# althonos/pyhmmer

Hardware: AMD Instinct MI355X
Metric: GCUPS (DP cells/s) + seqs/s for hmmsearch, Pfam-A vs proteome, 1/2/4/8 GPUs (higher is better)
Workload: dtype u8/i16 filters (MSV, Viterbi), f32 Forward/Backward

## Files before the change

### include/p7x.h

```cpp
#ifndef P7X_H
#define P7X_H

#include <stddef.h>
#include <stdint.h>

#ifdef __cplusplus
extern "C" {
#endif

#define P7X_ABI_VERSION 8

enum {
  P7X_OK = 0, P7X_EMEM = 5, P7X_EFORMAT = 7, P7X_EINVAL = 11, P7X_ERANGE = 16, P7X_ENORESULT = 19,
  P7X_ENODEVICE = 100, P7X_EDEVICE = 101
};

enum { P7X_RNA = 1, P7X_DNA = 2, P7X_AMINO = 3 };
enum { P7X_SEARCH_SEQS = 0, P7X_SCAN_MODELS = 1 };
enum { P7X_ZSETBY_NTARGETS = 0, P7X_ZSETBY_OPTION = 1, P7X_ZSETBY_FILEINFO = 2 };
enum { P7X_MMU = 0, P7X_MLAMBDA, P7X_VMU, P7X_VLAMBDA, P7X_FTAU, P7X_FLAMBDA };
enum { P7X_GA1 = 0, P7X_GA2, P7X_TC1, P7X_TC2, P7X_NC1, P7X_NC2 };
#define P7X_CUTOFF_UNSET (-99999.0f)
#define P7X_EVPARAM_UNSET (-99999.0f)
enum { P7X_IS_INCLUDED = 1, P7X_IS_REPORTED = 2, P7X_IS_NEW = 4, P7X_IS_DROPPED = 8, P7X_IS_DUPLICATE = 16 };
// ... 119 lines not shown
  int64_t seqidx;
  int32_t window_length;
  double sortkey;
  float score, pre_score, sum_score;
  double lnP, pre_lnP, sum_lnP;
  float nexpected;
  int32_t nregions, nclustered, noverlaps, nenvelopes, ndom;
  uint32_t flags;
  int32_t nreported, nincluded, best_domain;
} p7x_hit;

typedef struct p7x_tophits p7x_tophits;

int p7x_search_block(const p7x_pipeline_cfg *cfg, const p7x_oprofile *om, const float *bg_f,
                     const p7x_seqdb *db, const char *const *names, const char *const *accs,
                     const char *const *descs, p7x_tophits **out);

typedef struct p7x_pending p7x_pending;
int  p7x_search_block_begin(const p7x_pipeline_cfg *cfg, const p7x_oprofile *om, const float *bg_f,
                            const p7x_seqdb *db, p7x_pending **out);
int  p7x_search_block_finish(p7x_pending *pending, const char *const *names, const char *const *accs,
                             const char *const *descs, p7x_tophits **out);
void p7x_pending_destroy(p7x_pending *pending);
int  p7x_search_block_enqueue(const p7x_pipeline_cfg *cfg, const p7x_oprofile *om, const float *bg_f,
                              const p7x_seqdb *db, p7x_pending **out);
int  p7x_search_block_wait(p7x_pending *pending);
int  p7x_search_batch_enqueue(const p7x_pipeline_cfg *cfg, const p7x_oprofile *const *oms, size_t nq, const float *bg_f,
                              const p7x_seqdb *db, p7x_pending **out);
int  p7x_search_batch_finish(p7x_pending *pending, const char *const *names, const char *const *accs,
                             const char *const *descs, p7x_tophits **outs);
size_t p7x_pending_nqueries(const p7x_pending *pending);
int  p7x_debug_log_of_float(int device, const float *in, float *out, size_t n);
int  p7x_debug_memory_stats(int device, int64_t out[4]);
int  p7x_debug_choice(const float *p, int n, uint32_t x, int *via_thresholds, int *via_fchoose);
int  p7x_debug_order_spread(const p7x_oprofile *om, const uint8_t *dsq1, int32_t L, int32_t i, int32_t j, int multihit, double *out12);
int  p7x_debug_parser_rows(const p7x_oprofile *om, const uint8_t *dsq1, int32_t L, float *fx, float *bx);
int64_t p7x_debug_ssv_tables(const p7x_oprofile *om, int pair, int32_t *R, int32_t *pair_slack, uint32_t *tab4q, size_t cap_words);
int  p7x_debug_set_option(const char *name, int value);
int  p7x_debug_ensemble(const p7x_oprofile *om, const p7x_seqdb *db, int64_t target, int32_t i, int32_t j, uint32_t seed,
                        int use_device, int32_t *ndom, int32_t *dom, int32_t dom_cap, float *n2, int32_t *status);
int  p7x_search_batch_raw(const p7x_pipeline_cfg *cfg, const p7x_oprofile *const *oms, size_t nq, const float *bg_f,
                          const p7x_seqdb *db, int32_t *xJ, int32_t *xC, uint8_t *stage);

int p7x_search_longtargets(const p7x_pipeline_cfg *cfg, const p7x_oprofile *om, int device,
                           const uint8_t *dsq, const int64_t *offsets, const int64_t *lengths, size_t n,
                           const char *const *names, const char *const *accs, const char *const *descs, p7x_tophits **out);
int p7x_longtargets_release_resident(int device, uint64_t key);
int64_t p7x_ssv_longtarget_seeds(const p7x_pipeline_cfg *cfg, const p7x_oprofile *om, int device, const uint8_t *dsq, int64_t L,
                                 int complement, int64_t *seeds, size_t cap);
int p7x_longtarget_from_seeds(const p7x_pipeline_cfg *cfg, const p7x_oprofile *om,
                              const uint8_t *dsq, const int64_t *offsets, const int64_t *lengths, size_t n,
                              const char *const *names, const char *const *accs, const char *const *descs,
                              const int64_t *seed_target, const int64_t *seed_block, const int32_t *seed_strand,
                              const int64_t *seeds, size_t nseeds, p7x_tophits **out);

int p7x_forward_parser_exact(const p7x_oprofile *om, const uint8_t *dsq, int32_t L, float *sc);

int p7x_scan_collect(p7x_tophits *const *per_model, size_t nmodels, const p7x_pipeline_cfg *cfg, size_t nseqs,
                     const char *const *seq_names, const char *const *seq_accs, const char *const *seq_descs,
                     const int32_t *seq_lengths, p7x_tophits **out);
typedef struct p7x_scan_accum p7x_scan_accum;
int  p7x_scan_accum_create(const p7x_pipeline_cfg *cfg, size_t nseqs, const char *const *seq_names, const char *const *seq_accs,
                           const char *const *seq_descs, const int32_t *seq_lengths, p7x_scan_accum **out);
int  p7x_scan_accum_add(p7x_scan_accum *acc, p7x_tophits *const *per_model, size_t nmodels);
int  p7x_scan_accum_add_indexed(p7x_scan_accum *acc, p7x_tophits *const *per_model, const int64_t *model_index, size_t nmodels);
int  p7x_debug_tophits_set_stages(p7x_tophits *th, const uint8_t *stage, size_t n);
// ... 92 lines not shown
```

### pyhmmer_amd/_lib.py

```python
from __future__ import annotations

import ctypes as C
import os
import shutil
import subprocess
from pathlib import Path

_PKG = Path(__file__).resolve().parent
_ROOT = _PKG.parent
CSRC = _PKG / "csrc"
LIB_PATH = _PKG / "libp7x.so"

SOURCES = ["p7x_profile.cpp", "p7x_device.hip", "p7x_devmem.hip", "p7x_devimage.hip", "p7x_msv.hip", "p7x_vitfwd.hip", "p7x_vitpk.hip", "p7x_fwdpk.hip", "p7x_envelope.hip", "p7x_ensemble.hip", "p7x_ssvlong.hip", "p7x_longtarget.hip",
           "p7x_envscore.hip", "p7x_pipeline.hip", "p7x_domaindef.cpp", "p7x_longtarget_host.cpp", "p7x_tophits.cpp", "p7x_align.hip", "p7x_tracealign.cpp", "p7x_builder.cpp", "p7x_calibrate.hip"]


def _hipcc() -> str:
    for cand in (os.environ.get("HIPCC"), shutil.which("hipcc"), "/opt/rocm/bin/hipcc"):
        if cand and os.path.exists(cand):
            return cand
    raise RuntimeError("hipcc not found (need ROCm; set HIPCC=/path/to/hipcc)")


ISA_CHECKED = ("p7x_msv.hip", "p7x_envelope.hip")
# ... 163 lines not shown
    "p7x_pipeline_cfg_default": (None, [C.POINTER(PipelineCfg)]),
    "p7x_search_block": (C.c_int, [C.POINTER(PipelineCfg), _VP, _VP, _VP, _VP, _VP, _VP, C.POINTER(_VP)]),
    "p7x_postprocess_targets": (C.c_int, [C.POINTER(PipelineCfg), _VP, _VP, _VP, _VP, C.c_size_t, _VP, C.c_size_t, _VP, _VP, _VP,
                                          _VP, _VP, _VP, _VP, _VP, C.POINTER(_VP)]),
    "p7x_tophits_destroy": (None, [_VP]),
    "p7x_tophits_destroy_many": (None, [_VP, C.c_size_t]),
    "p7x_tophits_clone": (_VP, [_VP]),
    "p7x_tophits_nhits": (C.c_int64, [_VP]),
    "p7x_tophits_abc_type": (C.c_int, [_VP]),
    "p7x_tophits_get_counters": (C.c_int, [_VP, C.POINTER(Counters)]),
    "p7x_tophits_get_cfg": (C.c_int, [_VP, C.POINTER(PipelineCfg)]),
    "p7x_tophits_get_hit": (C.c_int, [_VP, C.c_int64, C.POINTER(HitRec)]),
    "p7x_tophits_get_domain": (C.c_int, [_VP, C.c_int64, C.c_int32, C.POINTER(DomainRec)]),
    "p7x_tophits_merge": (C.c_int, [_VP, _VP]),
    "p7x_tophits_serialize": (C.c_int64, [_VP, _VP, C.c_size_t]),
    "p7x_tophits_deserialize": (_VP, [_VP, C.c_size_t]),
    "p7x_tophits_sort_by_key": (C.c_int, [_VP]),
    "p7x_tophits_threshold": (C.c_int, [_VP]),
    "p7x_tophits_sort_by_seqidx": (C.c_int, [_VP]),
    "p7x_tophits_is_sorted": (C.c_int, [_VP, C.c_int]),
    "p7x_tophits_set_hit_flags": (C.c_int, [_VP, C.c_int64, C.c_uint32]),
    "p7x_tophits_set_hit_text": (C.c_int, [_VP, C.c_int64, C.c_int, C.c_char_p]),
    "p7x_tophits_get_timings": (C.c_int, [_VP, C.POINTER(C.c_double), C.c_int]),
    "p7x_search_block_begin": (C.c_int, [C.POINTER(PipelineCfg), _VP, _VP, _VP, C.POINTER(_VP)]),
    "p7x_search_block_enqueue": (C.c_int, [C.POINTER(PipelineCfg), _VP, _VP, _VP, C.POINTER(_VP)]),
    "p7x_search_block_wait": (C.c_int, [_VP]),
    "p7x_search_block_finish": (C.c_int, [_VP, _VP, _VP, _VP, C.POINTER(_VP)]),
    "p7x_pending_destroy": (None, [_VP]),
    "p7x_search_batch_enqueue": (C.c_int, [C.POINTER(PipelineCfg), C.POINTER(_VP), C.c_size_t, _VP, _VP, C.POINTER(_VP)]),
    "p7x_search_batch_finish": (C.c_int, [_VP, _VP, _VP, _VP, C.POINTER(_VP)]),
    "p7x_pending_nqueries": (C.c_size_t, [_VP]),
    "p7x_debug_log_of_float": (C.c_int, [C.c_int, _VP, _VP, C.c_size_t]),
    "p7x_debug_memory_stats": (C.c_int, [C.c_int, C.POINTER(C.c_int64)]),
    "p7x_debug_choice": (C.c_int, [_VP, C.c_int, C.c_uint32, _VP, _VP]),
    "p7x_debug_order_spread": (C.c_int, [_VP, _VP, C.c_int32, C.c_int32, C.c_int32, C.c_int, _VP]),
    "p7x_debug_parser_rows": (C.c_int, [_VP, _VP, C.c_int32, _VP, _VP]),
    "p7x_debug_ssv_tables": (C.c_int64, [_VP, C.c_int, _VP, _VP, _VP, C.c_size_t]),
    "p7x_debug_set_option": (C.c_int, [C.c_char_p, C.c_int]),
    "p7x_longtargets_release_resident": (C.c_int, [C.c_int, C.c_uint64]),
    "p7x_debug_ensemble": (C.c_int, [_VP, _VP, C.c_int64, C.c_int32, C.c_int32, C.c_uint32, C.c_int, _VP, _VP, C.c_int32, _VP, _VP]),
    "p7x_search_batch_raw": (C.c_int, [C.POINTER(PipelineCfg), C.POINTER(_VP), C.c_size_t, _VP, _VP, _VP, _VP, _VP]),
    "p7x_search_longtargets": (C.c_int, [C.POINTER(PipelineCfg), _VP, C.c_int, _VP, _VP, _VP, C.c_size_t, _VP, _VP, _VP, C.POINTER(_VP)]),
    "p7x_ssv_longtarget_seeds": (C.c_int64, [C.POINTER(PipelineCfg), _VP, C.c_int, _VP, C.c_int64, C.c_int, _VP, C.c_size_t]),
    "p7x_forward_parser_exact": (C.c_int, [_VP, _VP, C.c_int32, C.POINTER(C.c_float)]),
    "p7x_longtarget_from_seeds": (C.c_int, [C.POINTER(PipelineCfg), _VP, _VP, _VP, _VP, C.c_size_t, _VP, _VP, _VP, _VP, _VP, _VP, _VP,
                                            C.c_size_t, C.POINTER(_VP)]),
    "p7x_oprofile_write_pressed": (C.c_int, [_VP, C.POINTER(C.c_int64), _VP, C.c_size_t, C.POINTER(C.c_size_t), _VP, C.c_size_t,
                                             C.POINTER(C.c_size_t)]),
    "p7x_oprofile_read_pressed": (C.c_int, [_VP, C.c_size_t, _VP, C.c_size_t, _VP, C.POINTER(_VP), C.POINTER(C.c_size_t),
                                            C.POINTER(C.c_size_t), C.POINTER(C.c_int64)]),
    "p7x_oprofile_get_string": (C.c_int, [_VP, C.c_int, C.c_char_p, C.c_size_t]),
    "p7x_scan_collect": (C.c_int, [C.POINTER(_VP), C.c_size_t, C.POINTER(PipelineCfg), C.c_size_t, _VP, _VP, _VP, _VP, C.POINTER(_VP)]),
    "p7x_scan_accum_create": (C.c_int, [C.POINTER(PipelineCfg), C.c_size_t, _VP, _VP, _VP, _VP, C.POINTER(_VP)]),
    "p7x_scan_accum_add": (C.c_int, [_VP, C.POINTER(_VP), C.c_size_t]),
    "p7x_scan_accum_add_indexed": (C.c_int, [_VP, C.POINTER(_VP), C.POINTER(C.c_int64), C.c_size_t]),
    "p7x_debug_tophits_set_stages": (C.c_int, [_VP, _VP, C.c_size_t]),
    "p7x_scan_accum_finish": (C.c_int, [_VP, C.POINTER(_VP)]),
    "p7x_scan_accum_destroy": (None, [_VP]),
    "p7x_fasta_parse": (C.c_int, [_VP, C.c_size_t, _VP, C.POINTER(C.c_size_t), C.POINTER(C.c_size_t), C.POINTER(C.c_size_t),
                                  _VP, _VP, _VP, _VP, _VP, _VP, C.POINTER(C.c_size_t)]),
    "p7x_tracealign_compute": (C.c_int, [_VP, C.c_int, _VP, _VP, _VP, C.c_size_t, C.c_int, C.POINTER(_VP)]),
    "p7x_traces_count": (C.c_int64, [_VP]),
    "p7x_traces_nflagged": (C.c_int64, [_VP]),
    "p7x_traces_stats": (C.c_int, [_VP, _VP]),
    "p7x_traces_get": (C.c_int, [_VP, C.c_int64, C.POINTER(C.c_int32), C.POINTER(C.c_int32), C.POINTER(C.c_int32), _VP,
                                 C.POINTER(C.c_int32), C.POINTER(C.c_uint8)]),
# ... 64 lines not shown
```

### pyhmmer_amd/csrc/p7x_device.hip

```cpp
#include "p7x_device.hpp"
#include <cstdlib>
#include "p7x_kernels.hpp"
#include <algorithm>
#include <cmath>
#include <cstring>
#include <map>
#include <memory>

namespace p7x {

static std::mutex g_ctx_mu;
static std::map<int, std::unique_ptr<DeviceCtx>> g_ctx;

static int device_count_checked()
{
  int n = 0;
  if (hipGetDeviceCount(&n) != hipSuccess) { (void) hipGetLastError(); return 0; }
  return n;
}

static const int g_hw_queues_set = setenv("GPU_MAX_HW_QUEUES", "8", 0);

int create_tail_stream(DeviceCtx *ctx, bool high_priority, hipStream_t *out)
{
  (void) ctx;
  int least = 0, greatest = 0;
  P7X_HIP(hipDeviceGetStreamPriorityRange(&least, &greatest));
  P7X_HIP(hipStreamCreateWithPriority(out, hipStreamNonBlocking, high_priority ? greatest : least));
  return P7X_OK;
}

int get_ctx(int device, DeviceCtx **out)
{
  std::lock_guard<std::mutex> lk(g_ctx_mu);
  auto it = g_ctx.find(device);
  if (it != g_ctx.end()) { *out = it->second.get(); P7X_HIP(hipSetDevice(device)); return P7X_OK; }
  const int n = device_count_checked();
  if (device < 0 || device >= n) { set_error("no usable HIP device (libp7x has no CPU fallback)"); return P7X_ENODEVICE; }
  P7X_HIP(hipSetDevice(device));
  auto ctx = std::make_unique<DeviceCtx>();
  ctx->device = device;
  {
    int least = 0, greatest = 0;
    P7X_HIP(hipDeviceGetStreamPriorityRange(&least, &greatest));
    const int off[DeviceCtx::kWsSets] = { 0, 4, 2, 6 };
    int created = 0;
    for (int n = 0; n < DeviceCtx::kWsSets; ++n) {
      while (created % 8 != off[n]) { hipStream_t sp = nullptr; P7X_HIP(hipStreamCreateWithPriority(&sp, hipStreamNonBlocking, greatest)); ctx->ws_spacers.push_back(sp); ++created; }
      P7X_HIP(hipStreamCreateWithPriority(&ctx->ws_main[n], hipStreamNonBlocking, greatest)); ++created;
      for (auto &q : ctx->ws_side[n]) { P7X_HIP(hipStreamCreateWithPriority(&q, hipStreamNonBlocking, greatest)); ++created; }
    }
  }
  P7X_HIP(hipStreamCreateWithFlags(&ctx->stream, hipStreamNonBlocking));
  P7X_HIP(hipStreamCreateWithFlags(&ctx->stream2, hipStreamNonBlocking));
  for (auto &e : ctx->msv_done) P7X_HIP(hipEventCreateWithFlags(&e, hipEventDisableTiming));
  hipDeviceProp_t prop;
  P7X_HIP(hipGetDeviceProperties(&prop, device));
  ctx->num_cu = prop.multiProcessorCount;
  std::vector<uint8_t> tjb(kMaxL + 1);
  std::vector<int16_t> xwm(kMaxL + 1);
  std::vector<float> n1(kMaxL + 1);
  const float scale_b = 3.0 / kLog2, scale_w = 500.0 / kLog2;
  for (int L = 0; L <= kMaxL; ++L) {
    tjb[L] = unbiased_byteify(scale_b, logf(3.0f / (float) (L + 3)));
    const float pmove = (2.0f + 1.0f) / ((float) L + 2.0f + 1.0f);
    xwm[L] = wordify(scale_w, logf(pmove));
    n1[L] = null1_score(L);
  }
  P7X_HIP(hipMalloc(&ctx->lt.tjb, tjb.size()));
  P7X_HIP(hipMalloc(&ctx->lt.xwmove, xwm.size() * 2));
  P7X_HIP(hipMalloc(&ctx->lt.null1, n1.size() * 4));
  P7X_HIP(hipMemcpy(ctx->lt.tjb, tjb.data(), tjb.size(), hipMemcpyHostToDevice));
  P7X_HIP(hipMemcpy(ctx->lt.xwmove, xwm.data(), xwm.size() * 2, hipMemcpyHostToDevice));
  P7X_HIP(hipMemcpy(ctx->lt.null1, n1.data(), n1.size() * 4, hipMemcpyHostToDevice));
  {
    std::vector<double> lt(256);
    for (int i = 0; i < 128; ++i) { const double c = 1.0 + ((double) i + 0.5) / 128.0; lt[2 * i] = 1.0 / c; lt[2 * i + 1] = std::log(c); }
    P7X_HIP(hipMalloc(&ctx->lt.logtab, lt.size() * 8));
    P7X_HIP(hipMemcpy(ctx->lt.logtab, lt.data(), lt.size() * 8, hipMemcpyHostToDevice));
  }
  *out = ctx.get();
// ... 8 lines not shown
  const int g = blockIdx.x;
  const int lane = threadIdx.x & 63;
  const int wave = threadIdx.x >> 6, nwave = blockDim.x >> 6;
  const int64_t slot = (int64_t) g * 64 + lane;
  const int L = slot < nslots ? slot_len[slot] : 0;
  const uint8_t *src = slot < nslots ? dsq + slot_off[slot] : dsq;
  const int nblk = grp_nblk[g];
  uint4 *dst = tiles + grp_off[g] + lane;
  for (int b = wave; b < nblk; b += nwave) {
    uint32_t w[4];
#pragma unroll
    for (int q = 0; q < 4; ++q) {
      uint32_t acc = 0;
#pragma unroll
      for (int r = 0; r < 4; ++r) {
        const int i = b * 16 + q * 4 + r;
        const uint32_t x = (i < L) ? src[i] : (uint32_t) pad;
        acc |= x << (8 * r);
      }
      w[q] = acc;
    }
    dst[(size_t) b * 64] = make_uint4(w[0], w[1], w[2], w[3]);
  }
}

}

using namespace p7x;

extern "C" {

int p7x_device_count(void) { return device_count_checked(); }

int p7x_device_name(int device, char *buf, size_t n)
{
  if (!buf || n == 0) return P7X_EINVAL;
  if (device < 0 || device >= device_count_checked()) { set_error("no such device"); return P7X_ENODEVICE; }
  hipDeviceProp_t prop;
  P7X_HIP(hipGetDeviceProperties(&prop, device));
  std::snprintf(buf, n, "%s (%s, %d CUs)", prop.name, prop.gcnArchName, prop.multiProcessorCount);
  return P7X_OK;
}

int p7x_seqdb_create(int device, int32_t abc_type, const uint8_t *dsq, const int64_t *offsets,
                     const int32_t *lengths, size_t n, p7x_seqdb **out)
{
  if (!out || (n && (!dsq || !offsets || !lengths))) { set_error("p7x_seqdb_create: bad arguments"); return P7X_EINVAL; }
  DeviceCtx *ctx = nullptr;
  int st = get_ctx(device, &ctx);
  if (st != P7X_OK) return st;
  auto db = std::make_unique<p7x_seqdb>();
  db->device = device; db->abc_type = abc_type; db->Kp = Alphabet::get(abc_type).Kp; db->n = (int64_t) n;
  db->h_len.assign(lengths, lengths + n);
  db->h_off.resize(n);
  int maxL = 0; int64_t nres = 0, nslots = 0;
  for (size_t t = 0; t < n; ++t) {
    if (lengths[t] < 0) { set_error("negative target length"); return P7X_EINVAL; }
    if (lengths[t] > kMaxL) { set_error("Target sequence length > 100K, over comparison pipeline limit"); return P7X_ERANGE; }
    nres += lengths[t]; if (lengths[t] > 0) ++nslots; if (lengths[t] > maxL) maxL = lengths[t];
  }
  db->nres = nres; db->nslots = nslots; db->ngroups = (nslots + 63) / 64;
  db->h_dsq.assign((size_t) nres + n + 1, 255);
  {
    int64_t pos = 1;
    for (size_t t = 0; t < n; ++t) {
      db->h_off[t] = pos;
// ... 80 lines not shown
```

### pyhmmer_amd/csrc/p7x_device.hpp

```cpp
#pragma once
#include "p7x_internal.hpp"
#include "p7x_devmem.hpp"
#include <hip/hip_runtime.h>
#include <map>
#include <memory>
#include <mutex>

namespace p7x {

constexpr int kMaxL      = 100000;
constexpr int kTabRows   = 32;
constexpr int kNegPad    = -512;

#define P7X_HIP(call)                                                                          \
  do { hipError_t e_ = (call); if (e_ != hipSuccess) {                                         \
    p7x::set_error(std::string(#call) + ": " + hipGetErrorString(e_)); return e_ == hipErrorOutOfMemory ? P7X_EMEM : P7X_EDEVICE; } } while (0)

struct LengthTables {
  uint8_t *tjb = nullptr;
  int16_t *xwmove = nullptr;
  float   *null1 = nullptr;
  double  *logtab = nullptr;
};

struct DeviceCtx {
  int device = -1;
  hipStream_t stream = nullptr;
  hipStream_t stream2 = nullptr;
  LengthTables lt;
  int num_cu = 256;
  std::mutex mu;
  std::mutex msv_mu;
  std::mutex lt_scan_mu;
  static constexpr int kLtStreams = 4;
  hipStream_t lt_stream[kLtStreams]{};
  int lt_next = 0;
  hipEvent_t msv_done[2] = { nullptr, nullptr };
  int msv_last = -1;
  std::mutex slab_mu;
  std::multimap<size_t, void *> slab_free;
  size_t slab_free_bytes = 0;
  size_t slab_obtained_bytes = 0;
  static constexpr int kWsSets = 4, kWsSide = 7;
  hipStream_t ws_main[kWsSets]{};
  hipStream_t ws_side[kWsSets][kWsSide]{};
  std::vector<hipStream_t> ws_spacers;
  int ws_set_users[kWsSets]{};
};
int get_ctx(int device, DeviceCtx **out);
int create_tail_stream(DeviceCtx *ctx, bool high_priority, hipStream_t *out);

struct DevProfile {
  int device = -1;
  int M = 0, Kp = 0;
  int msvR = 0, msvK = 0, msvS = 0;
  uint32_t *msv_tab = nullptr;
  int16_t *msvw_emis = nullptr;
  uint32_t *msvw_pk = nullptr;
  int msvwC = 0, msvw_rows = kTabRows;
  int vitC = 0, Mpad = 0;
  int16_t *vit_trans = nullptr;
  int16_t *vit_emis = nullptr;
  int vitpkT = 0, vitpkP = 0;
  uint32_t *vitpk_trans = nullptr, *vitpk_emis = nullptr;
  float *fwd_trans = nullptr;
  float *fwd_emis = nullptr;
  int fwdgT = 0, fwdgC = 0;
  float *fwdg_trans = nullptr, *fwdg_emis = nullptr;
  float *bias_eo = nullptr;
  std::shared_ptr<DeviceBuf> shared;
};

int get_dev_profile(const p7x_oprofile *om, DeviceCtx *ctx, DevProfile **out);
int get_dev_profiles(const p7x_oprofile *const *oms, int n, DeviceCtx *ctx, DevProfile **out, int nthreads);
void free_dev_profile(DevProfile *d);

struct EnvelopeScorer;
struct EnsembleRunner;
}
struct p7x_seqdb;
#include <memory>
namespace p7x {
// ... 33 lines not shown
```

### pyhmmer_amd/csrc/p7x_internal.hpp

```cpp
#pragma once
#include "../../include/p7x.h"
#include <cstdint>
#include <string>
#include <vector>

namespace p7x {

constexpr int MAXK  = 20;
constexpr int MAXKP = 29;
constexpr double kLog2  = 0.69314718055994529;
constexpr double kLog2R = 1.44269504088896341;

enum { XE = 0, XN = 1, XJ = 2, XC = 3 };
enum { MOVE = 0, LOOP = 1 };
enum { tBM = 0, tMM, tIM, tDM, tMD, tMI, tII, tDD, NTRANS };
enum { gMM = 0, gIM, gDM, gBM, gMD, gDD, gMI, gII };

struct Alphabet {
  int type, K, Kp;
  const char *sym;
  unsigned char degen[MAXKP][MAXK];
  static const Alphabet &get(int type);
};

// ... 7 lines not shown
  std::vector<float> tsc;
  std::vector<float> msc;
  float xsc[4][2];
  std::vector<uint8_t> rb;
  uint8_t tbm_b, tec_b, tjb_b, base_b, bias_b;
  float scale_b;
  std::vector<int16_t> rw;
  std::vector<int16_t> tw;
  int16_t xw[4][2];
  float scale_w; int16_t base_w, ddbound_w; float ncj_roundoff;
  std::vector<float> rf_;
  std::vector<float> tf;
  float xf[4][2];

  int Q16() const { int q = (M - 1) / 16 + 1; return q < 2 ? 2 : q; }
  int Q8()  const { int q = (M - 1) / 8  + 1; return q < 2 ? 2 : q; }
  int Q4()  const { int q = (M - 1) / 4  + 1; return q < 2 ? 2 : q; }
};

float  sse_expf(float x);
uint8_t unbiased_byteify(float scale_b, float sc);
int16_t wordify(float scale_w, float sc);
double gumbel_surv(double x, double mu, double lambda);
double exp_surv(double x, double mu, double lambda);
double exp_logsurv(double x, double mu, double lambda);
float  null1_score(int L);
double match_relent_sum(const float *mat, const float *bg_f, int M, int K);
void   flogsum_init();
float  flogsum(float a, float b);

void set_error(const std::string &msg);

enum { OPT_SMALL_BLOCK = 0, OPT_VIT_WAVE, OPT_MSV_EXACT, OPT_MSV_LONG_GROUPS, OPT_MSV_BLOCKS_PER_CU, OPT_ENV_WORKSPACE_GB, OPT_DEVICE_CLUSTERED,
       OPT_TRACE_FINISH, OPT_TRACE_LONGTARGET, OPT_TRACE_ENVELOPE, OPT_HOST_PROFILE, OPT_SSV_KERNEL, OPT_MSV_F16, OPT_ENS_LDS_KB, OPT_ENS_FAIL, OPT_MSV_TIERS, OPT_STAGE_MERGE, OPT_EARLY_PACK, OPT_HOST_ORDER, OPT_VIT_LONG_CUT, OPT_FWD_GROUPED, OPT_REGION_GUARD_PPM, OPT_MSV_K8, OPT_MSV_LANE_BLOCKS, OPT_HOST_ALIGN, OPT_ALIGN_WORKSPACE_GB, OPT_COUNT };
int debug_opt(int which);

}
struct p7x_oprofile;
namespace p7x {
void attach_dev_cache(p7x_oprofile *om);

}

struct p7x_oprofile { p7x::Profile p; void *dev_cache = nullptr; };
```

### pyhmmer_amd/csrc/p7x_pipeline.hip

```cpp
#include "p7x_wave.hpp"
#include "p7x_host.hpp"
#include <atomic>
#include <chrono>
#include <cmath>
#include <cstdlib>
#include <cstring>
#include <memory>
#include <string>

namespace p7x {

struct StageBufs {
  int16_t *xJ;
  float *usc, *filtersc, *vfsc, *fwdsc;
  int32_t *xC;
  float *fwd_by_item;
  int32_t *list_bias, *list_vit, *list_fwd, *list_fin;
  uint8_t *stage;
  int *counters;
};

struct StageParams {
  double F1, F2, F3;
  double F3_near;
// ... 419 lines not shown
    }
  }
}

struct LaneArgs {
  DecideArgs dec;
  MsvArgs msv, msv_amb;
  MsvWaveArgs msvw;
  VitPkArgs vitpk;
  CompactArgs cmp;
  WaveSeqArgs vit, fwd, rows, bck;
  LayoutArgs lay;
  RegionArgs reg;
};
constexpr int kLaneCounters = 16;

struct Workspace {
  int device = -1; DeviceCtx *ctx = nullptr; int64_t cap_slots = 0; int nlanes = 0;
  DeviceBuf xJ , usc, filtersc, vfsc, fwdsc , xC , fwd_by_item ;
  DeviceBuf list_bias, list_vit, list_fwd, list_fin;
  DeviceBuf stage;
  DeviceBuf chunk_cnt; int64_t chunks_per_lane = 0;
  DeviceBuf counters;
  DeviceBuf d_args; PinnedBuf h_args;
  DeviceBuf xmx_f, xmx_b, xmx_s; int64_t xmx_cap = 0;
  DeviceBuf xmx_off , reg_out , bck_sc ;
  int64_t fin_cap = 0;
  DeviceBuf rt_xmx_off, rt_reg_out, rt_bck_sc; int64_t rt_cap = 0;
  hipEvent_t ev[8]{};
  hipEvent_t ev_sync = nullptr;
  hipStream_t stream = nullptr;
  static constexpr int kSide = DeviceCtx::kWsSide;
  hipStream_t side[kSide]{};
  hipEvent_t ev_fork = nullptr, ev_join[kSide]{};
  static constexpr int kTierRuns = 8;
  hipEvent_t ev_tier[kTierRuns]{}, ev_tier0[kTierRuns]{};
  int ntier_runs = 0, tier_lanes[kTierRuns]{}; int64_t tier_nodes[kTierRuns]{};
  PinnedBuf h_counts;
  DeviceBuf pack_dev; PinnedBuf pack_host;
  int64_t early_T_cap = 0;
  int64_t last_T = 2048;
  int set = -1;
  size_t counters_bytes() const { return (size_t) nlanes * kLaneCounters * 4 + 8; }
  unsigned long long *cursor() const { return reinterpret_cast<unsigned long long *>(counters.as<int>() + (size_t) nlanes * kLaneCounters); }
  ~Workspace() {
    if (device < 0) return;
    (void) hipSetDevice(device);
    for (auto &e : ev) if (e) (void) hipEventDestroy(e);
    if (ev_sync) (void) hipEventDestroy(ev_sync);
    if (ev_fork) (void) hipEventDestroy(ev_fork);
    for (auto &e : ev_join) if (e) (void) hipEventDestroy(e);
    for (auto &e : ev_tier) if (e) (void) hipEventDestroy(e);
    for (auto &e : ev_tier0) if (e) (void) hipEventDestroy(e);
  }
  StageBufs lane_bufs(int l) const
  {
    const size_t o = (size_t) l * (size_t) cap_slots;
    StageBufs b{};
    b.xJ = xJ.as<int16_t>() + o; b.usc = usc.as<float>() + o; b.filtersc = filtersc.as<float>() + o; b.vfsc = vfsc.as<float>() + o; b.fwdsc = fwdsc.as<float>() + o;
    b.xC = xC.as<int32_t>() + o; b.fwd_by_item = fwd_by_item.as<float>() + o;
    b.list_bias = list_bias.as<int32_t>() + o; b.list_vit = list_vit.as<int32_t>() + o; b.list_fwd = list_fwd.as<int32_t>() + o; b.list_fin = list_fin.as<int32_t>() + o;
    b.stage = stage.as<uint8_t>() + o; b.counters = counters.as<int>() + (size_t) l * kLaneCounters;
    return b;
  }
  void take_stream_set()
  {
    std::lock_guard<std::mutex> lk(ctx->mu);
    set = 0;
    for (int k = 1; k < DeviceCtx::kWsSets; ++k) if (ctx->ws_set_users[k] < ctx->ws_set_users[set]) set = k;
    ctx->ws_set_users[set]++;
    stream = ctx->ws_main[set];
    for (int k = 0; k < kSide; ++k) side[k] = ctx->ws_side[set][k];
  }
  void on_return()
  {
    if (set < 0) return;
    std::lock_guard<std::mutex> lk(ctx->mu);
    if (ctx->ws_set_users[set] > 0) ctx->ws_set_users[set]--;
    set = -1;
  }
};

static int build_workspace(Workspace *w, DeviceCtx *ctx, int64_t nslots, int nlanes)
{
  w->ctx = ctx; w->nlanes = nlanes;
  const int64_t cap = std::max<int64_t>(64, ((nslots + 63) / 64) * 64);
  const size_t tot = (size_t) cap * (size_t) nlanes;
  w->chunks_per_lane = (cap + kCompactChunk - 1) / kCompactChunk;
  const std::pair<DeviceBuf *, size_t> dev[] = {
    { &w->xJ, tot * 2 }, { &w->usc, tot * 4 }, { &w->filtersc, tot * 4 }, { &w->vfsc, tot * 4 }, { &w->fwdsc, tot * 4 }, { &w->xC, tot * 4 },
    { &w->fwd_by_item, tot * 4 }, { &w->list_bias, tot * 4 }, { &w->list_vit, tot * 4 }, { &w->list_fwd, tot * 4 }, { &w->list_fin, tot * 4 },
    { &w->counters, w->counters_bytes() }, { &w->d_args, (size_t) nlanes * sizeof(LaneArgs) }, { &w->stage, tot },
    { &w->chunk_cnt, (size_t) nlanes * (size_t) w->chunks_per_lane * 4 } };
  int st = P7X_OK;
  for (const auto &d : dev) if ((st = d.first->reserve(ctx, d.second)) != P7X_OK) return st;
  if ((st = w->h_counts.reserve(w->counters_bytes())) != P7X_OK || (st = w->h_args.reserve((size_t) nlanes * sizeof(LaneArgs))) != P7X_OK) return st;
  for (auto &e : w->ev) P7X_HIP(hipEventCreate(&e));
  P7X_HIP(hipEventCreateWithFlags(&w->ev_sync, hipEventDisableTiming));
  P7X_HIP(hipEventCreateWithFlags(&w->ev_fork, hipEventDisableTiming));
  for (auto &e : w->ev_join) P7X_HIP(hipEventCreateWithFlags(&e, hipEventDisableTiming));
  for (auto &e : w->ev_tier) P7X_HIP(hipEventCreate(&e));
  for (auto &e : w->ev_tier0) P7X_HIP(hipEventCreate(&e));
  w->cap_slots = cap;
  return P7X_OK;
}
// ... 491 lines not shown
    for (size_t n = 0; n < runs.size(); ++n)
      if ((st = class_viterbi(runs[n], r.lm, ctx, ws, stream_of(n))) != P7X_OK) return st;
  }
  if ((st = join()) != P7X_OK) return st;
  hipLaunchKernelGGL(decide_vit_kernel, dim3(lane_grid((r.est_vit + 255) / 256, ctx->num_cu, nq), (unsigned) nq), dim3(256), 0, s, dec);
  P7X_HIP(hipEventRecord(ws->ev[3], s));
  const std::vector<LaneClass> by_C = runs_by([](const LaneClass &a, const LaneClass &b) { return a.C == b.C; });
  if ((st = fork()) != P7X_OK) return st;
  for (size_t n = 0; n < by_C.size(); ++n)
    if ((st = class_wave(by_C[n], ws, &LaneArgs::fwd, false, ctx, stream_of(n))) != P7X_OK) return st;
  if ((st = join()) != P7X_OK) return st;
  hipLaunchKernelGGL(decide_fwd_kernel, dim3(lane_grid((r.est_fwd + 255) / 256, ctx->num_cu, nq), (unsigned) nq), dim3(256), 0, s, dec);
  P7X_HIP(hipEventRecord(ws->ev[4], s));
  hipLaunchKernelGGL(layout_rows_kernel, dim3(1, (unsigned) nq), dim3(256), 0, s, lane_run(ws, &LaneArgs::lay, 0, nq).ref());
  P7X_HIP(hipGetLastError());
  P7X_HIP(hipEventRecord(ws->ev[5], s));
  if ((st = fork()) != P7X_OK) return st;
  for (size_t n = 0; n < by_C.size(); ++n) {
    hipStream_t cs = stream_of(n);
    if ((st = class_wave(by_C[n], ws, &LaneArgs::rows, false, ctx, cs)) != P7X_OK) return st;
    if ((st = class_wave(by_C[n], ws, &LaneArgs::bck, true, ctx, cs)) != P7X_OK) return st;
  }
  if ((st = join()) != P7X_OK) return st;
  {
    const int64_t items = std::min<int64_t>(ws->fin_cap, std::max(r.est_fin, 1));
    const unsigned gx = lane_grid((items + 3) / 4, ctx->num_cu * 4, nq);
    hipLaunchKernelGGL(regions_kernel, dim3(gx, (unsigned) nq), dim3(256), 0, s, lane_run(ws, &LaneArgs::reg, 0, nq).ref());
    P7X_HIP(hipGetLastError());
  }
  P7X_HIP(hipEventRecord(ws->ev[6], s));
  return P7X_OK;
}

static int cascade_enqueue(CascadeRun &r)
{
  const p7x_pipeline_cfg &cfg = r.cfg; const p7x_seqdb *db = r.db;
  int st = get_ctx(db->device, &r.ctx);
  if (st != P7X_OK) return st;
  DeviceCtx *ctx = r.ctx;
  const int nq = (int) r.oms.size();
  r.query_of.resize(nq);
  for (int i = 0; i < nq; ++i) r.query_of[i] = i;
  std::stable_sort(r.query_of.begin(), r.query_of.end(), [&](int a, int b) { return r.oms[a]->p.M < r.oms[b]->p.M; });
  r.lane_of.resize(nq); r.lm.resize(nq);
  for (int l = 0; l < nq; ++l) { r.lane_of[r.query_of[l]] = l; r.lm[l].om = r.oms[r.query_of[l]]; }
  const bool debug = debug_opt(OPT_TRACE_FINISH) > 0;
  auto tlast = std::chrono::steady_clock::now();
  std::string dbg;
  auto tick = [&](const char *what) {
    if (!debug) return;
    const auto now = std::chrono::steady_clock::now();
    char buf[64]; std::snprintf(buf, sizeof buf, " %s %.2f", what, std::chrono::duration<double, std::milli>(now - tlast).count());
    dbg += buf; tlast = now;
  };
  {
    std::vector<const p7x_oprofile *> lane_oms((size_t) nq);
    std::vector<DevProfile *> dps((size_t) nq, nullptr);
    for (int l = 0; l < nq; ++l) lane_oms[(size_t) l] = r.lm[l].om;
    if ((st = get_dev_profiles(lane_oms.data(), nq, ctx, dps.data(), cfg.host_threads)) != P7X_OK) return st;
    for (int l = 0; l < nq; ++l) r.lm[l].dp = dps[(size_t) l];
  }
  tick("images");
  if (db->nslots == 0 || nq == 0) return P7X_OK;
  for (int l = 0; l < nq; ++l)
    if (r.lm[l].dp->vitC <= 0) { set_error("model too long for the device kernels: M > 8192 nodes (the reference has no limit, plan7.pyx:6156-6262; the lane-chunk layout of the wave-per-target kernels ends at 128 nodes per lane -- no Pfam-A model comes near it)"); return P7X_EINVAL; }
  std::vector<LaneClass> classes;
// ... 12 lines not shown
    const Profile &p = r.lm[l].om->p; const DevProfile *dp = r.lm[l].dp;
    LaneArgs &la = ws->h_args.as<LaneArgs>()[l];
    const StageBufs b = ws->lane_bufs(l);
    DecideArgs d{};
    d.b = b; d.p = make_params(p, cfg);
    d.slot_len = db->d_slot_len; d.tjb_tab = ctx->lt.tjb; d.null1_tab = ctx->lt.null1; d.xwmove_tab = ctx->lt.xwmove; d.logtab = ctx->lt.logtab;
    d.dsq = db->d_dsq; d.slot_off = db->d_slot_off; d.eo = dp->bias_eo; d.nslots = db->nslots;
    la.dec = d;
    fill_msv_args(la, p, dp, db, ctx, b, nlong_of[(size_t) l]);
    const int64_t vit_long = vit_long_of[(size_t) l];
    fill_vit_args(la, p, dp, db, ctx, b.list_vit, est.vit, &b.counters[2], b.xC,
                  vit_long > 0 ? &b.counters[13] : nullptr, (int) std::min<int64_t>(vit_long, (int64_t) est.vit));
    CompactArgs ca{};
    ca.stage = b.stage; ca.list = b.list_vit; ca.chunk_cnt = ws->chunk_cnt.as<int>() + (size_t) l * (size_t) ws->chunks_per_lane; ca.counters = b.counters;
    ca.nslots = db->nslots; ca.long_slots = vit_long;
    la.cmp = ca;
    WaveSeqArgs a = ws_args(p, dp, db, ctx);
    a.trans = dp->fwd_trans; a.emis = dp->fwd_emis; a.list = b.list_fwd; a.nlist = est.fwd; a.nlist_ptr = &b.counters[3];
    a.out_sc = b.fwd_by_item;
    if (fwd_grouped(db) && dp->fwdgT > 0) { a.trans = dp->fwdg_trans; a.emis = dp->fwdg_emis; a.C = dp->fwdgT * 256 + dp->fwdgC; a.counter = &b.counters[5]; }
    la.fwd = a;
  }
  tick("args");
  if ((st = fill_survivor_args(r, 0, nq, false, 0)) != P7X_OK) return st;
  tick("survivor_args");
  if ((st = upload_args(ws, 0, nq, s)) != P7X_OK) return st;
  tick("upload");
  P7X_HIP(hipMemsetAsync(ws->counters.as<int>(), 0, ws->counters_bytes(), s));
  ws->ntier_runs = 0;
  if (classes.size() == 1) {
    const bool fills_device = (db->nslots / 64) * (int64_t) nq >= (int64_t) ctx->num_cu * 8;
    if ((st = class_cascade(r, classes[0], s, true, fills_device)) != P7X_OK) return st;
  } else {
    P7X_HIP(hipEventRecord(ws->ev_fork, s));
    const int nside = std::min<int>((int) classes.size() - 1, Workspace::kSide);
    for (int k = 0; k < nside; ++k) P7X_HIP(hipStreamWaitEvent(ws->side[k], ws->ev_fork, 0));
    constexpr int kStreamsAll = Workspace::kSide + 1;
    std::vector<int> run_of(classes.size(), -1);
    if (msv_tiers_enabled()) {
      int nruns = 0, last_tier = -1;
      for (size_t c = 0; c < classes.size(); ++c) {
        const LaneClass &k = classes[c];
        if (k.msv_key < 0) { last_tier = -1; continue; }
        const int tier = msv_tier(r.lm[k.first].dp->msvR, r.lm[k.first].dp->msvK);
        if (tier != last_tier) { if (nruns == Workspace::kTierRuns) break; ++nruns; last_tier = tier; }
        run_of[c] = nruns - 1;
      }
      for (int run = nruns - 1; run >= 0; --run) {
        size_t a = 0; while (run_of[a] != run) ++a;
        size_t b = a; while (b + 1 < classes.size() && run_of[b + 1] == run) ++b;
        const int first = classes[a].first, n = classes[b].first + classes[b].n - first;
        const int turn = (kStreamsAll - 1 - run) % kStreamsAll;
        hipStream_t ts = turn == 0 ? s : ws->side[std::min(turn, nside) - 1];
        const LaneClass &k = classes[a];
        P7X_HIP(hipEventRecord(ws->ev_tier0[run], ts));
        if ((st = msv_tier_launch(msv_tier(r.lm[k.first].dp->msvR, r.lm[k.first].dp->msvK), lane_run(ws, &LaneArgs::msv, first, n), ctx->num_cu, ts)) != P7X_OK) return st;
        P7X_HIP(hipEventRecord(ws->ev_tier[run], ts));
        ws->tier_lanes[run] = n; ws->tier_nodes[run] = 0;
        for (int l = first; l < first + n; ++l) ws->tier_nodes[run] += r.lm[l].om->p.M;
      }
      ws->ntier_runs = nruns;
    }
    const int sm = debug_opt(OPT_STAGE_MERGE);
    const bool staged = sm >= 0 ? sm != 0 : db->ngroups <= 256;
    if (staged) {
      if ((st = staged_cascade(r, classes, s, nside, run_of)) != P7X_OK) return st;
    } else
    for (size_t n = 0; n < classes.size(); ++n) {
      const size_t c = classes.size() - 1 - n;
      constexpr int kStreams = Workspace::kSide + 1;
      int turn = (int) (n % (size_t) kStreams);
      if ((n / (size_t) kStreams) & 1) turn = kStreams - 1 - turn;
      hipStream_t cs = turn == 0 ? s : ws->side[turn - 1];
      if (run_of[c] >= 0) P7X_HIP(hipStreamWaitEvent(cs, ws->ev_tier[run_of[c]], 0));
      if ((st = class_cascade(r, classes[c], cs, n == 0, false, run_of[c] >= 0)) != P7X_OK) return st;
    }
    for (int k = 0; k < nside; ++k) {
      P7X_HIP(hipEventRecord(ws->ev_join[k], ws->side[k]));
      P7X_HIP(hipStreamWaitEvent(s, ws->ev_join[k], 0));
    }
  }
  ws->early_T_cap = 0;
  if (debug_opt(OPT_EARLY_PACK) > 0 || (debug_opt(OPT_EARLY_PACK) < 0 && db->ngroups <= 256)) {
    int64_t room = 1024;
    while (room < 16384 && room < 2 * ws->last_T) room *= 2;
    const int64_t kEarlyPack = debug_opt(OPT_EARLY_PACK) > 0 ? debug_opt(OPT_EARLY_PACK) : room;
    const PackLayout lay = pack_layout(nq, kEarlyPack, cfg.mode == P7X_SCAN_MODELS, db->nslots);
    if ((st = queue_pack(r, lay, kEarlyPack, nullptr, 2048)) != P7X_OK) return st;
    ws->early_T_cap = kEarlyPack;
  }
  P7X_HIP(hipMemcpyAsync(ws->h_counts.as<int>(), ws->counters.as<int>(), ws->counters_bytes(), hipMemcpyDeviceToHost, s));
  P7X_HIP(hipEventRecord(ws->ev_sync, s));
  tick("launches");
  if (debug) std::fprintf(stderr, "[enqueue] nq %d classes %zu:%s ms\n", nq, classes.size(), dbg.c_str());
  return P7X_OK;
}

static int retry_survivor_passes(CascadeRun &r, int l, int nfin)
{
  Workspace *ws = r.ws.get(); hipStream_t s = ws->stream;
  int st = fill_survivor_args(r, l, 1, true, nfin);
  if (st != P7X_OK) return st;
  if ((st = upload_args(ws, l, 1, s)) != P7X_OK) return st;
  P7X_HIP(hipMemsetAsync(&ws->lane_bufs(l).counters[12], 0, 4, s));
  P7X_HIP(hipMemsetAsync(ws->cursor(), 0, 8, s));
  LaneClass c; c.first = l; c.n = 1; c.C = r.lm[l].dp->vitC;
  if ((st = launch_survivor_passes(r, c, s, true, false)) != P7X_OK) return st;
  P7X_HIP(hipMemcpyAsync(ws->h_counts.as<int>(), ws->counters.as<int>(), ws->counters_bytes(), hipMemcpyDeviceToHost, s));
  P7X_HIP(hipEventRecord(ws->ev_sync, s));
  return P7X_OK;
}

// ... 609 lines not shown
```

### pyhmmer_amd/csrc/p7x_profile.cpp

```cpp
#include "p7x_internal.hpp"
#include <atomic>
#include <algorithm>
#include <cmath>
#include <cstdio>
#include <cstring>
#include <memory>
#include <mutex>

namespace p7x {
std::atomic<int> g_debug_opt[OPT_COUNT];
static const bool g_debug_opt_ready = [] { for (auto &o : g_debug_opt) o.store(-1); return true; }();
int debug_opt(int which) { return (which >= 0 && which < OPT_COUNT) ? g_debug_opt[which].load(std::memory_order_relaxed) : -1; }


static thread_local std::string g_err;
void set_error(const std::string &msg) { g_err = msg; }

static Alphabet make_alphabet(int type)
{
  Alphabet a{};
  a.type = type;
  std::memset(a.degen, 0, sizeof(a.degen));
  if (type == P7X_AMINO) {
    a.K = 20; a.Kp = 29; a.sym = "ACDEFGHIKLMNPQRSTVWY-BJZOUX*~";
// ... 197 lines not shown
{
  const int M = p.M;
  p.rf_.assign((size_t) p.Kp * (M + 1), 0.0f);
  for (int x = 0; x < p.Kp; ++x)
    for (int k = 1; k <= M; ++k) p.rf_[(size_t) x * (M + 1) + k] = sse_expf(p.msc[(size_t) x * (M + 1) + k]);
  p.tf.assign((size_t) NTRANS * (M + 1), 0.0f);
  auto F = [&](int t, int k) -> float & { return p.tf[(size_t) t * (M + 1) + k]; };
  for (int k = 1; k <= M; ++k) {
    F(tBM, k) = sse_expf(p.tsc[(size_t) (k - 1) * 8 + gBM]);
    F(tMM, k) = sse_expf(p.tsc[(size_t) (k - 1) * 8 + gMM]);
    F(tIM, k) = sse_expf(p.tsc[(size_t) (k - 1) * 8 + gIM]);
    F(tDM, k) = sse_expf(p.tsc[(size_t) (k - 1) * 8 + gDM]);
    if (k < M) {
      F(tMD, k) = sse_expf(p.tsc[(size_t) k * 8 + gMD]);
      F(tMI, k) = sse_expf(p.tsc[(size_t) k * 8 + gMI]);
      F(tII, k) = sse_expf(p.tsc[(size_t) k * 8 + gII]);
      F(tDD, k) = sse_expf(p.tsc[(size_t) k * 8 + gDD]);
    }
  }
  for (int s = 0; s < 4; ++s) for (int m = 0; m < 2; ++m) p.xf[s][m] = expf(p.xsc[s][m]);
}

}

using namespace p7x;

extern "C" {

int p7x_abi_version(void) { return P7X_ABI_VERSION; }

int p7x_debug_set_option(const char *name, int value)
{
  static const char *const names[p7x::OPT_COUNT] = { "small_block", "vit_wave", "msv_exact", "msv_long_groups", "msv_blocks_per_cu", "env_workspace_gb",
                                                     "device_clustered", "trace_finish", "trace_longtarget", "trace_envelope", "host_profile", "ssv_kernel", "msv_f16", "ens_lds_kb", "ens_fail", "msv_tiers", "stage_merge", "early_pack", "host_order", "vit_long_cut", "fwd_grouped", "region_guard_ppm", "msv_k8", "msv_lane_blocks", "host_align", "align_workspace_gb" };
  if (!name) { p7x::set_error("p7x_debug_set_option: no name"); return P7X_EINVAL; }
  for (int i = 0; i < p7x::OPT_COUNT; ++i)
    if (std::strcmp(name, names[i]) == 0) { p7x::g_debug_opt[i].store(value); return P7X_OK; }
  p7x::set_error(std::string("p7x_debug_set_option: unknown option ") + name);
  return P7X_EINVAL;
}

const char *p7x_last_error(void) { return g_err.c_str(); }

void p7x_expf_neg(const double *in, float *out, size_t n)
{
  for (size_t i = 0; i < n; ++i) out[i] = std::isinf(in[i]) ? 0.0f : expf((float) (-1.0 * in[i]));
}

int p7x_hmm_max_length(const p7x_hmm_view *h, double beta, int32_t *out)
{
  if (!h || !out || h->M < 1 || !h->t || !(beta > 0.0)) { set_error("p7x_hmm_max_length: bad arguments"); return P7X_EINVAL; }
  const int M = h->M;
  if (M == 1) { *out = 1; return P7X_OK; }
  const float *t = h->t;
  auto T = [&](int k, int x) -> double { return (double) t[(size_t) k * 7 + x]; };
  std::vector<double> Mm(2 * (size_t) (M + 1), 0.0), I(2 * (size_t) (M + 1), 0.0), D(2 * (size_t) (M + 1), 0.0);
  auto at = [&](std::vector<double> &v, int k, int c) -> double & { return v[(size_t) c * (M + 1) + k]; };
  at(Mm, 1, 0) = 1.0;
  for (int k = 2; k <= M; ++k) at(D, k, 0) = T(k - 1, 2) * at(Mm, k - 1, 0) + T(k - 1, 6) * at(D, k - 1, 0);
  const int length_bound = 200000;
  for (int L = 2; L <= length_bound; ++L) {
    const int c = (L - 1) & 1, pc = L & 1;
    at(Mm, 1, c) = 0.0; at(D, 1, c) = 0.0;
    at(I, 1, c) = T(1, 1) * at(Mm, 1, pc) + T(1, 4) * at(I, 1, pc);
    double alive = at(I, 1, c);
    for (int k = 2; k <= M; ++k) {
      const double m = T(k - 1, 0) * at(Mm, k - 1, pc) + T(k - 1, 3) * at(I, k - 1, pc) + T(k - 1, 5) * at(D, k - 1, pc);
// ... 380 lines not shown
```

Measured before the change: 23800.

## Limit non-staged cascade to two streams and remap stream-to-hardware-queue placement

Result: faster. 25920 (median of 6 runs) (+8.9%).

```diff
diff --git a/include/p7x.h b/include/p7x.h
--- a/include/p7x.h
+++ b/include/p7x.h
@@ -175,6 +175,7 @@
 size_t p7x_pending_nqueries(const p7x_pending *pending);
 int  p7x_debug_log_of_float(int device, const float *in, float *out, size_t n);
 int  p7x_debug_memory_stats(int device, int64_t out[4]);
+int64_t p7x_debug_stream_plan(int32_t *out, size_t cap, int32_t *hw_queues);
 int  p7x_debug_choice(const float *p, int n, uint32_t x, int *via_thresholds, int *via_fchoose);
 int  p7x_debug_order_spread(const p7x_oprofile *om, const uint8_t *dsq1, int32_t L, int32_t i, int32_t j, int multihit, double *out12);
 int  p7x_debug_parser_rows(const p7x_oprofile *om, const uint8_t *dsq1, int32_t L, float *fx, float *bx);
diff --git a/pyhmmer_amd/_lib.py b/pyhmmer_amd/_lib.py
--- a/pyhmmer_amd/_lib.py
+++ b/pyhmmer_amd/_lib.py
@@ -219,6 +219,7 @@
     "p7x_pending_nqueries": (C.c_size_t, [_VP]),
     "p7x_debug_log_of_float": (C.c_int, [C.c_int, _VP, _VP, C.c_size_t]),
     "p7x_debug_memory_stats": (C.c_int, [C.c_int, C.POINTER(C.c_int64)]),
+    "p7x_debug_stream_plan": (C.c_int64, [C.POINTER(C.c_int32), C.c_size_t, C.POINTER(C.c_int32)]),
     "p7x_debug_choice": (C.c_int, [_VP, C.c_int, C.c_uint32, _VP, _VP]),
     "p7x_debug_order_spread": (C.c_int, [_VP, _VP, C.c_int32, C.c_int32, C.c_int32, C.c_int, _VP]),
     "p7x_debug_parser_rows": (C.c_int, [_VP, _VP, C.c_int32, _VP, _VP]),
diff --git a/pyhmmer_amd/csrc/p7x_device.hip b/pyhmmer_amd/csrc/p7x_device.hip
--- a/pyhmmer_amd/csrc/p7x_device.hip
+++ b/pyhmmer_amd/csrc/p7x_device.hip
@@ -19,7 +19,24 @@
   return n;
 }
 
+static const char *const g_hw_queues_env = std::getenv("GPU_MAX_HW_QUEUES");
+static const int g_hw_queues_seen = !g_hw_queues_env ? 0 : (std::atoi(g_hw_queues_env) > 0 ? std::atoi(g_hw_queues_env) : -1);
 static const int g_hw_queues_set = setenv("GPU_MAX_HW_QUEUES", "8", 0);
+
+StreamPlan stream_plan(int nsets, int per_set)
+{
+  StreamPlan p;
+  p.nsets = nsets; p.per_set = per_set;
+  p.partner = 4 - 1;
+  int next = 0;
+  while (next < 8) p.spacer_pos.push_back(next++);
+  for (int n = 0; n < nsets; ++n) {
+    while (next % 8 != n % 8) p.spacer_pos.push_back(next++);
+    p.main_pos.push_back(next);
+    next += per_set;
+  }
+  return p;
+}
 
 int create_tail_stream(DeviceCtx *ctx, bool high_priority, hipStream_t *out)
 {
@@ -43,10 +60,11 @@
   {
     int least = 0, greatest = 0;
     P7X_HIP(hipDeviceGetStreamPriorityRange(&least, &greatest));
-    const int off[DeviceCtx::kWsSets] = { 0, 4, 2, 6 };
+    const StreamPlan plan = stream_plan(DeviceCtx::kWsSets, DeviceCtx::kWsSide + 1);
+    ctx->ws_partner = plan.partner;
     int created = 0;
     for (int n = 0; n < DeviceCtx::kWsSets; ++n) {
-      while (created % 8 != off[n]) { hipStream_t sp = nullptr; P7X_HIP(hipStreamCreateWithPriority(&sp, hipStreamNonBlocking, greatest)); ctx->ws_spacers.push_back(sp); ++created; }
+      while (created < plan.main_pos[(size_t) n]) { hipStream_t sp = nullptr; P7X_HIP(hipStreamCreateWithPriority(&sp, hipStreamNonBlocking, greatest)); ctx->ws_spacers.push_back(sp); ++created; }
       P7X_HIP(hipStreamCreateWithPriority(&ctx->ws_main[n], hipStreamNonBlocking, greatest)); ++created;
       for (auto &q : ctx->ws_side[n]) { P7X_HIP(hipStreamCreateWithPriority(&q, hipStreamNonBlocking, greatest)); ++created; }
     }
@@ -121,6 +139,17 @@
 
 int p7x_device_count(void) { return device_count_checked(); }
 
+int64_t p7x_debug_stream_plan(int32_t *out, size_t cap, int32_t *hw_queues)
+{
+  const StreamPlan p = stream_plan(DeviceCtx::kWsSets, DeviceCtx::kWsSide + 1);
+  std::vector<int32_t> v = { p.nsets, p.per_set, p.partner, (int32_t) p.spacer_pos.size() };
+  for (int n = 0; n < p.nsets; ++n) for (int k = 0; k < p.per_set; ++k) v.push_back(p.main_pos[(size_t) n] + k);
+  v.insert(v.end(), p.spacer_pos.begin(), p.spacer_pos.end());
+  if (out && cap >= v.size()) std::copy(v.begin(), v.end(), out);
+  if (hw_queues) *hw_queues = g_hw_queues_seen;
+  return (int64_t) v.size();
+}
+
 int p7x_device_name(int device, char *buf, size_t n)
 {
   if (!buf || n == 0) return P7X_EINVAL;
diff --git a/pyhmmer_amd/csrc/p7x_device.hpp b/pyhmmer_amd/csrc/p7x_device.hpp
--- a/pyhmmer_amd/csrc/p7x_device.hpp
+++ b/pyhmmer_amd/csrc/p7x_device.hpp
@@ -44,10 +44,18 @@
   static constexpr int kWsSets = 4, kWsSide = 7;
   hipStream_t ws_main[kWsSets]{};
   hipStream_t ws_side[kWsSets][kWsSide]{};
+  int ws_partner = 0;
   std::vector<hipStream_t> ws_spacers;
   int ws_set_users[kWsSets]{};
 };
 int get_ctx(int device, DeviceCtx **out);
+struct StreamPlan {
+  int nsets = 0, per_set = 0;
+  int partner = 0;
+  std::vector<int> main_pos;
+  std::vector<int> spacer_pos;
+};
+StreamPlan stream_plan(int nsets, int per_set);
 int create_tail_stream(DeviceCtx *ctx, bool high_priority, hipStream_t *out);
 
 struct DevProfile {
diff --git a/pyhmmer_amd/csrc/p7x_internal.hpp b/pyhmmer_amd/csrc/p7x_internal.hpp
--- a/pyhmmer_amd/csrc/p7x_internal.hpp
+++ b/pyhmmer_amd/csrc/p7x_internal.hpp
@@ -63,7 +63,7 @@
 void set_error(const std::string &msg);
 
 enum { OPT_SMALL_BLOCK = 0, OPT_VIT_WAVE, OPT_MSV_EXACT, OPT_MSV_LONG_GROUPS, OPT_MSV_BLOCKS_PER_CU, OPT_ENV_WORKSPACE_GB, OPT_DEVICE_CLUSTERED,
-       OPT_TRACE_FINISH, OPT_TRACE_LONGTARGET, OPT_TRACE_ENVELOPE, OPT_HOST_PROFILE, OPT_SSV_KERNEL, OPT_MSV_F16, OPT_ENS_LDS_KB, OPT_ENS_FAIL, OPT_MSV_TIERS, OPT_STAGE_MERGE, OPT_EARLY_PACK, OPT_HOST_ORDER, OPT_VIT_LONG_CUT, OPT_FWD_GROUPED, OPT_REGION_GUARD_PPM, OPT_MSV_K8, OPT_MSV_LANE_BLOCKS, OPT_HOST_ALIGN, OPT_ALIGN_WORKSPACE_GB, OPT_COUNT };
+       OPT_TRACE_FINISH, OPT_TRACE_LONGTARGET, OPT_TRACE_ENVELOPE, OPT_HOST_PROFILE, OPT_SSV_KERNEL, OPT_MSV_F16, OPT_ENS_LDS_KB, OPT_ENS_FAIL, OPT_MSV_TIERS, OPT_STAGE_MERGE, OPT_EARLY_PACK, OPT_HOST_ORDER, OPT_VIT_LONG_CUT, OPT_FWD_GROUPED, OPT_REGION_GUARD_PPM, OPT_MSV_K8, OPT_MSV_LANE_BLOCKS, OPT_HOST_ALIGN, OPT_ALIGN_WORKSPACE_GB, OPT_CASCADE_STREAMS, OPT_CASCADE_SPLIT, OPT_COUNT };
 int debug_opt(int which);
 
 }
diff --git a/pyhmmer_amd/csrc/p7x_pipeline.hip b/pyhmmer_amd/csrc/p7x_pipeline.hip
--- a/pyhmmer_amd/csrc/p7x_pipeline.hip
+++ b/pyhmmer_amd/csrc/p7x_pipeline.hip
@@ -475,6 +475,7 @@
   hipStream_t stream = nullptr;
   static constexpr int kSide = DeviceCtx::kWsSide;
   hipStream_t side[kSide]{};
+  int partner = 0;
   hipEvent_t ev_fork = nullptr, ev_join[kSide]{};
   static constexpr int kTierRuns = 8;
   hipEvent_t ev_tier[kTierRuns]{}, ev_tier0[kTierRuns]{};
@@ -514,6 +515,7 @@
     ctx->ws_set_users[set]++;
     stream = ctx->ws_main[set];
     for (int k = 0; k < kSide; ++k) side[k] = ctx->ws_side[set][k];
+    partner = ctx->ws_partner;
   }
   void on_return()
   {
@@ -1071,6 +1073,8 @@
   return P7X_OK;
 }
 
+constexpr int kCascadeStreams = 2;
+
 static int cascade_enqueue(CascadeRun &r)
 {
   const p7x_pipeline_cfg &cfg = r.cfg; const p7x_seqdb *db = r.db;
@@ -1149,9 +1153,17 @@
     const bool fills_device = (db->nslots / 64) * (int64_t) nq >= (int64_t) ctx->num_cu * 8;
     if ((st = class_cascade(r, classes[0], s, true, fills_device)) != P7X_OK) return st;
   } else {
+    const int sm = debug_opt(OPT_STAGE_MERGE);
+    const bool staged = sm >= 0 ? sm != 0 : db->ngroups <= 256;
+    const int cs_opt = debug_opt(OPT_CASCADE_STREAMS);
+    const int nstreams = staged ? Workspace::kSide + 1 : (cs_opt == 1 || cs_opt == 2 || cs_opt == 8 ? cs_opt : kCascadeStreams);
+    const bool few = nstreams < Workspace::kSide + 1;
+    const bool split = nstreams == 2 && debug_opt(OPT_CASCADE_SPLIT) > 0;
+    hipStream_t partner = ws->side[ws->partner];
     P7X_HIP(hipEventRecord(ws->ev_fork, s));
     const int nside = std::min<int>((int) classes.size() - 1, Workspace::kSide);
-    for (int k = 0; k < nside; ++k) P7X_HIP(hipStreamWaitEvent(ws->side[k], ws->ev_fork, 0));
+    if (!few) for (int k = 0; k < nside; ++k) P7X_HIP(hipStreamWaitEvent(ws->side[k], ws->ev_fork, 0));
+    else if (nstreams == 2) P7X_HIP(hipStreamWaitEvent(partner, ws->ev_fork, 0));
     constexpr int kStreamsAll = Workspace::kSide + 1;
     std::vector<int> run_of(classes.size(), -1);
     if (msv_tiers_enabled()) {
@@ -1168,7 +1180,7 @@
         size_t b = a; while (b + 1 < classes.size() && run_of[b + 1] == run) ++b;
         const int first = classes[a].first, n = classes[b].first + classes[b].n - first;
         const int turn = (kStreamsAll - 1 - run) % kStreamsAll;
-        hipStream_t ts = turn == 0 ? s : ws->side[std::min(turn, nside) - 1];
+        hipStream_t ts = few ? s : (turn == 0 ? s : ws->side[std::min(turn, nside) - 1]);
         const LaneClass &k = classes[a];
         P7X_HIP(hipEventRecord(ws->ev_tier0[run], ts));
         if ((st = msv_tier_launch(msv_tier(r.lm[k.first].dp->msvR, r.lm[k.first].dp->msvK), lane_run(ws, &LaneArgs::msv, first, n), ctx->num_cu, ts)) != P7X_OK) return st;
@@ -1178,8 +1190,6 @@
       }
       ws->ntier_runs = nruns;
     }
-    const int sm = debug_opt(OPT_STAGE_MERGE);
-    const bool staged = sm >= 0 ? sm != 0 : db->ngroups <= 256;
     if (staged) {
       if ((st = staged_cascade(r, classes, s, nside, run_of)) != P7X_OK) return st;
     } else
@@ -1189,12 +1199,16 @@
       int turn = (int) (n % (size_t) kStreams);
       if ((n / (size_t) kStreams) & 1) turn = kStreams - 1 - turn;
       hipStream_t cs = turn == 0 ? s : ws->side[turn - 1];
+      if (few) cs = nstreams == 1 ? s : (split || (n & 1) ? partner : s);
       if (run_of[c] >= 0) P7X_HIP(hipStreamWaitEvent(cs, ws->ev_tier[run_of[c]], 0));
       if ((st = class_cascade(r, classes[c], cs, n == 0, false, run_of[c] >= 0)) != P7X_OK) return st;
     }
-    for (int k = 0; k < nside; ++k) {
+    if (!few) for (int k = 0; k < nside; ++k) {
       P7X_HIP(hipEventRecord(ws->ev_join[k], ws->side[k]));
       P7X_HIP(hipStreamWaitEvent(s, ws->ev_join[k], 0));
+    } else if (nstreams == 2) {
+      P7X_HIP(hipEventRecord(ws->ev_join[ws->partner], partner));
+      P7X_HIP(hipStreamWaitEvent(s, ws->ev_join[ws->partner], 0));
     }
   }
   ws->early_T_cap = 0;
diff --git a/pyhmmer_amd/csrc/p7x_profile.cpp b/pyhmmer_amd/csrc/p7x_profile.cpp
--- a/pyhmmer_amd/csrc/p7x_profile.cpp
+++ b/pyhmmer_amd/csrc/p7x_profile.cpp
@@ -253,7 +253,7 @@
 int p7x_debug_set_option(const char *name, int value)
 {
   static const char *const names[p7x::OPT_COUNT] = { "small_block", "vit_wave", "msv_exact", "msv_long_groups", "msv_blocks_per_cu", "env_workspace_gb",
-                                                     "device_clustered", "trace_finish", "trace_longtarget", "trace_envelope", "host_profile", "ssv_kernel", "msv_f16", "ens_lds_kb", "ens_fail", "msv_tiers", "stage_merge", "early_pack", "host_order", "vit_long_cut", "fwd_grouped", "region_guard_ppm", "msv_k8", "msv_lane_blocks", "host_align", "align_workspace_gb" };
+                                                     "device_clustered", "trace_finish", "trace_longtarget", "trace_envelope", "host_profile", "ssv_kernel", "msv_f16", "ens_lds_kb", "ens_fail", "msv_tiers", "stage_merge", "early_pack", "host_order", "vit_long_cut", "fwd_grouped", "region_guard_ppm", "msv_k8", "msv_lane_blocks", "host_align", "align_workspace_gb", "cascade_streams", "cascade_split" };
   if (!name) { p7x::set_error("p7x_debug_set_option: no name"); return P7X_EINVAL; }
   for (int i = 0; i < p7x::OPT_COUNT; ++i)
     if (std::strcmp(name, names[i]) == 0) { p7x::g_debug_opt[i].store(value); return P7X_OK; }
```
